# FrozenWolf-Cyber/Indic-CL-ASR

Measured on AMD Instinct MI355X. Metric: utterances/sec (15 s @16 kHz) Conformer-M RNNT-CTC+EWC train step, higher is better.
Workload: dtype bf16; 1 GPU; BASELINE configs[1]: Conformer-medium (d=256, 16L, H=640) hybrid RNNT-CTC + EWC, bs=32/GPU x 15 s, bf16 projections, freeze_encoder_till=12, 22x257 heads, fused_batch_size=4; global_batch=32, parallelism=dp1

## Files before the change

include/indicasr.h:

```cpp
#ifndef INDICASR_H
#define INDICASR_H

#include <stddef.h>
#include <stdint.h>

#ifdef __cplusplus
extern "C" {
#endif

typedef void* ia_stream_t;

enum ia_status {
    IA_OK = 0,
    IA_INVALID_VALUE = -1,
    IA_WORKSPACE_TOO_SMALL = -2,
    IA_LAUNCH_FAILED = -3,
    IA_UNSUPPORTED = -4,
};

const char* ia_version(void);

size_t ia_rnnt_workspace_bytes(int B, int T, int U1);
int ia_rnnt_loss(const float* logits, const int64_t* labels, const int64_t* act_lens, const int64_t* label_lens,
                 int B, int T, int U1, int V, int blank, float fastemit_lambda, float clamp,
// ... 6 lines not shown
                     const float* cost_grad, float* grads, void* workspace, size_t workspace_bytes, ia_stream_t stream,
                     void* grad_kernel_start_event, void* grad_kernel_stop_event);
int ia_rnnt_export_alphas_betas(const void* workspace, size_t workspace_bytes, const int64_t* act_lens,
                                const int64_t* label_lens, int B, int T, int U1, float* alphas, float* betas,
                                ia_stream_t stream);

int ia_joint_ld(int V);
int ia_joint_fwd(const void* f, const void* g, const void* W, const float* bias, const int64_t* labels,
                 const int64_t* act_lens, const int64_t* label_lens, int B, int T, int U1, int H, int V, int blank,
                 float dropout_p, unsigned seed, void* logits, int LD, void* workspace, size_t workspace_bytes,
                 ia_stream_t stream);
int ia_joint_fwd_box(const void* f, const void* g, const void* W, const float* bias, const int64_t* labels,
                     const int64_t* act_lens, const int64_t* label_lens, const int64_t* box_t, const int64_t* box_u, int B,
                     int T, int U1, int H, int V, int blank, float dropout_p, unsigned seed, void* logits, int LD,
                     void* workspace, size_t workspace_bytes, ia_stream_t stream);
int64_t ia_joint_extra_scratch_elems(void);
int ia_joint_extra_reduce(const void* logits, const void* teacher, const int64_t* box_t, const int64_t* box_u,
                          const float* w_sq, const float* w_kd, int B, int T, int U1, int V, int LD, float* sums4,
                          float* scratch, ia_stream_t stream);
int ia_joint_extra_grad(const void* logits, const void* teacher, const int64_t* box_t, const int64_t* box_u, const float* w_sq,
                        const float* w_kd, const float* upstream2, int B, int T, int U1, int V, int LD, void* E,
                        ia_stream_t stream);
int ia_lattice_add_f16(void* G, const void* E, int64_t n, ia_stream_t stream);
int ia_rnnt_lattice(const int64_t* act_lens, const int64_t* label_lens, int B, int T, int U1, float fastemit_lambda,
                    int need_backward, float* costs, void* workspace, size_t workspace_bytes, ia_stream_t stream);
int ia_joint_backward_g(void* logits_inout, const int64_t* labels, const int64_t* act_lens, const int64_t* label_lens,
                        int B, int T, int U1, int V, int LD, int blank, float fastemit_lambda, const float* cost_grad,
                        float kappa, void* gt_out, int S, int Kc, float* dbias_out, float* dbias_scratch, void* workspace,
                        size_t workspace_bytes, ia_stream_t stream, void* grad_kernel_start_event,
                        void* grad_kernel_stop_event);
int ia_joint_backward_g_skip(void* logits_inout, const int64_t* labels, const int64_t* act_lens, const int64_t* label_lens, int B,
                             int T, int U1, int V, int LD, int blank, float fastemit, const float* cost_grad, float kappa,
                             void* gt_out, int S, int Kc, float* dbias_out, float* dbias_scratch, void* workspace,
                             size_t workspace_bytes, int skip_dead_frames, ia_stream_t stream, void* ev_start, void* ev_stop);
int64_t ia_joint_backward_g_dbias_scratch_elems(int LD);
int ia_joint_hidden_t(const void* f, const void* g, void* hidden_t, int B, int T, int U1, int H, int LDH, int S, int Kc,
                      float dropout_p, unsigned seed, ia_stream_t stream);
int ia_joint_hidden(const void* f, const void* g, void* hidden, int B, int T, int U1, int H, int LDH, float dropout_p,
                    unsigned seed, ia_stream_t stream);
int ia_joint_dh_reduce(const void* dh, const void* f, const void* g, const int64_t* act_lens,
                       const int64_t* label_lens, float* df, float* dg, int B, int T, int U1, int H, float inv_kappa,
                       float dropout_p, unsigned seed, void* scratch, ia_stream_t stream);
size_t ia_joint_dh_reduce_scratch_bytes(int B, int T, int U1, int H);
int ia_joint_dh_fused_supported(int U1, int H, int LD);
int ia_joint_dh_k(void);
size_t ia_joint_dh_fused_scratch_bytes(int B, int T, int U1, int H);
int ia_joint_dh_fused(const void* G, const void* Wt, const void* f, const void* g, const int64_t* act_lens,
                      const int64_t* label_lens, float* df, float* dg, int B, int T, int U1, int H, int LD,
                      float inv_kappa, float dropout_p, unsigned seed, void* scratch, ia_stream_t stream);
int ia_joint_dh_fused_ex(const void* G, const void* Wt, const void* f, const void* g, const int64_t* act_lens,
                         const int64_t* label_lens, float* df, float* dg, void* df_bf16, void* dg_bf16, int zero_dead_df, int B,
                         int T, int U1, int H, int LD, float inv_kappa, float dropout_p, unsigned seed, void* scratch,
                         ia_stream_t stream);
int ia_joint_dw_fused_supported(int U1, int H, int LD);
int64_t ia_joint_dw_fused_scratch_elems(int B, int T, int U1, int H, int LD);
int ia_joint_dw_fused(const void* G, const void* f, const void* g, const int64_t* act_lens, int B, int T, int U1, int H, int LD,
                      float dropout_p, unsigned seed, float* dW, float* scratch, ia_stream_t stream);
int ia_joint_dw_fused_ex(const void* G, const void* f, const void* g, const int64_t* act_lens, const int64_t* label_lens, int B,
                         int T, int U1, int H, int LD, float dropout_p, unsigned seed, float* dW, float* scratch,
                         ia_stream_t stream);

int ia_gemm_bf16(const void* A, int lda, const void* W, int ldw, int M, int N, int K, const float* bias, int act,
                 float dropout_p, unsigned seed, float alpha, const float* R, int ldr, float* outF, int ldof,
                 void* outH, int ldoh, ia_stream_t stream);
int ia_gemm_bf16_ex(const void* A, int lda, const void* W, int ldw, int M, int N, int K, const float* bias, int act,
                    float dropout_p, unsigned seed, float alpha, const float* R, int ldr, float* outF, int ldof, void* outH,
                    int ldoh, void* out_pre, int ldpre, const void* aux, int ldaux, ia_stream_t stream);
int ia_gemm_bf16_ex2(const void* A, int lda, const void* W, int ldw, int M, int N, int K, const float* bias, int act,
                     float dropout_p, unsigned seed, float alpha, const float* R, int ldr, float* outF, int ldof, void* outH,
                     int ldoh, void* out_pre, int ldpre, const void* aux, int ldaux, int flags, ia_stream_t stream);
int ia_quantize_mxfp8(const void* x, int is_f32, int ld, int64_t M, int K, void* q, int ldq, void* scales, int lds, ia_stream_t stream);
int ia_gemm_mxfp8(const void* Aq, int lda, const void* a_scales, int ldsa, const void* Wq, int ldw, const void* w_scales, int ldsw,
                  int M, int N, int K, const float* bias, int act, float dropout_p, unsigned seed, float alpha, const float* R, int ldr,
                  float* outF, int ldof, void* outH, int ldoh, ia_stream_t stream);

int ia_greedy_decode_lds_bytes(int Hp, int Hj, int V);
int ia_greedy_rnnt_decode(const float* f_all, const int64_t* out_len, const float* EW, const float* Whh, const float* Wpred,
                          const float* bpred, const float* Whead, const float* bhead, int B, int T, int Hp, int Hj, int V,
                          int blank, int row_blank, int row_sos, int max_symbols, int* tokens, int cap, int* counts,
                          int* overflow, ia_stream_t stream);
int ia_greedy_rnnt_decode_bf16w(const float* f_all, const int64_t* out_len, const float* EW, const void* Whh_bf16,
                                const void* Wpred_bf16, const float* bpred, const void* Whead_bf16, const float* bhead, int B, int T,
                                int Hp, int Hj, int V, int blank, int row_blank, int row_sos, int max_symbols, int* tokens, int cap,
                                int* counts, int* overflow, ia_stream_t stream);
size_t ia_greedy_decode_scratch_bytes(int B, int Hp, int Hj);
int ia_greedy_decode_cluster(int B, int Hp, int Hj);
int ia_greedy_rnnt_decode_bf16w_ex(const float* f_all, const int64_t* out_len, const float* EW, const void* Whh_bf16,
                                   const void* Wpred_bf16, const float* bpred, const void* Whead_bf16, const float* bhead, int B,
                                   int T, int Hp, int Hj, int V, int blank, int row_blank, int row_sos, int max_symbols, int* tokens,
                                   int cap, int* counts, int* overflow, int cluster, void* scratch, size_t scratch_bytes,
                                   ia_stream_t stream);

int ia_edit_distance_batch(const int32_t* a, const int64_t* a_off, const int32_t* b, const int64_t* b_off, int n, int64_t* out);

int ia_quantize_fp8_rows(const void* x, int is_f32, int ld, int64_t M, int K, void* q, int ldq, float* scale, ia_stream_t stream);
int ia_gemm_fp8(const void* Aq, int lda, const float* a_scale, const void* Wq, int ldw, const float* w_scale, int M, int N, int K,
                const float* bias, int act, float dropout_p, unsigned seed, float alpha, const float* R, int ldr, float* outF,
                int ldof, void* outH, int ldoh, ia_stream_t stream);
int ia_subsample_conv1(const float* feats, int B, int Fm, int Tm, int C, const float* w1, const float* b1, void* out,
                       ia_stream_t stream);
int ia_subsample_conv2(const void* in_cl, int B, int T1, int F1, int C, const void* w2r, const float* b2, int N, void* out,
                       ia_stream_t stream);
int ia_gemm_bf16_ln_supported(int N, int K);
int ia_gemm_bf16_ln(const void* A, int lda, const void* W, int ldw, int M, int N, int K, const float* bias, float dropout_p,
                    unsigned seed, float alpha, const float* R, int ldr, float* outF, int ldof, const float* ln_g,
                    const float* ln_b, float ln_eps, void* outH, int ldoh, ia_stream_t stream);
// ... 450 lines not shown
```

indic_cl_asr_amd/_lib.py:

```python
import ctypes
import os
import subprocess

_HERE = os.path.dirname(os.path.abspath(__file__))
LIB_PATH = os.environ.get("IA_LIB_PATH") or os.path.join(_HERE, "libindicasr_hip.so")

IA_OK = 0
_STATUS = {-1: "IA_INVALID_VALUE", -2: "IA_WORKSPACE_TOO_SMALL", -3: "IA_LAUNCH_FAILED", -4: "IA_UNSUPPORTED"}

_c = ctypes
_vp, _i, _f, _sz = _c.c_void_p, _c.c_int, _c.c_float, _c.c_size_t
_i64 = _c.c_int64

class BlockParams(_c.Structure):
    _fields_ = ([(n, _c.c_void_p) for n in (
        "w_ff1a", "w_ff1b", "w_qkv", "w_pos", "w_out", "w_pw1", "w_pw2", "w_ff2a", "w_ff2b",
        "b_ff1a", "b_ff1b", "b_qkv", "b_out", "b_pw1", "b_pw2", "b_ff2a", "b_ff2b",
        "ln_ff1_g", "ln_ff1_b", "ln_att_g", "ln_att_b", "ln_conv_g", "ln_conv_b", "ln_ff2_g", "ln_ff2_b", "ln_out_g", "ln_out_b",
        "pos_u", "pos_v", "dw_w", "dw_b", "bn_g", "bn_b", "bn_rm", "bn_rv", "bn_nbt")]
        + [(n, _c.c_float) for n in ("ln_eps", "bn_eps", "bn_momentum", "p_drop", "p_ff", "p_att", "fc_factor")]
        + [(n, _c.c_int) for n in ("d", "d_ff", "n_heads", "ksz")]
        + [("pl_cached", _c.c_void_p), ("w_pw1_glu", _c.c_void_p), ("b_pw1_glu", _c.c_void_p), ("att_window", _c.c_int),
           ("att_style", _c.c_int), ("att_left", _c.c_int), ("att_right", _c.c_int)])

# ... 52 lines not shown
    "ia_rnnt_backward": (_i, [_vp, _vp, _vp, _vp, _i, _i, _i, _i, _i, _f, _f, _vp, _vp, _vp, _sz, _vp, _vp, _vp]),
    "ia_rnnt_export_alphas_betas": (_i, [_vp, _sz, _vp, _vp, _i, _i, _i, _vp, _vp, _vp]),
    "ia_joint_ld": (_i, [_i]),
    "ia_joint_fwd": (_i, [_vp, _vp, _vp, _vp, _vp, _vp, _vp, _i, _i, _i, _i, _i, _i, _f, _c.c_uint, _vp, _i, _vp, _sz, _vp]),
    "ia_joint_fwd_box": (_i, [_vp, _vp, _vp, _vp, _vp, _vp, _vp, _vp, _vp, _i, _i, _i, _i, _i, _i, _f, _c.c_uint, _vp, _i, _vp, _sz, _vp]),
    "ia_joint_extra_scratch_elems": (_i64, []),
    "ia_joint_extra_reduce": (_i, [_vp, _vp, _vp, _vp, _vp, _vp, _i, _i, _i, _i, _i, _vp, _vp, _vp]),
    "ia_joint_extra_grad": (_i, [_vp, _vp, _vp, _vp, _vp, _vp, _vp, _i, _i, _i, _i, _i, _vp, _vp]),
    "ia_lattice_add_f16": (_i, [_vp, _vp, _i64, _vp]),
    "ia_relpos_attention_flash_lse": (_i, [_vp, _vp, _vp, _vp, _vp, _i, _i, _i, _i, _f, _c.c_uint, _vp, _vp, _vp]),
    "ia_relpos_attention_flash_bwd_dims": (_i, [_i, _c.POINTER(_c.c_int), _c.POINTER(_c.c_int)]),
    "ia_relpos_attention_flash_bwd_ws_elems": (_i64, [_i, _i, _i, _i]),
    "ia_relpos_attention_flash_bwd": (_i, [_vp, _vp, _vp, _vp, _vp, _vp, _vp, _vp, _i, _i, _i, _i, _f, _c.c_uint, _vp, _vp, _i, _vp,
                                           _vp, _vp, _vp, _vp, _vp]),
    "ia_relpos_attention_local_lse": (_i, [_vp, _vp, _vp, _vp, _vp, _i, _i, _i, _i, _i, _f, _c.c_uint, _vp, _vp, _vp]),
    "ia_relpos_attention_local_bwd_dims": (_i, [_i, _i, _c.POINTER(_c.c_int), _c.POINTER(_c.c_int)]),
    "ia_relpos_attention_local_bwd_ws_elems": (_i64, [_i, _i, _i, _i, _i]),
    "ia_relpos_attention_local_bwd": (_i, [_vp, _vp, _vp, _vp, _vp, _vp, _vp, _vp, _i, _i, _i, _i, _i, _f, _c.c_uint, _vp, _vp, _i, _vp,
                                           _vp, _vp, _vp, _vp, _vp]),
    "ia_relpos_attention_context_lse": (_i, [_vp, _vp, _vp, _vp, _vp, _i, _i, _i, _i, _i, _i, _i, _f, _c.c_uint, _vp, _vp, _vp]),
    "ia_relpos_attention_context_bwd_dims": (_i, [_i, _i, _i, _i, _c.POINTER(_c.c_int), _c.POINTER(_c.c_int)]),
    "ia_relpos_attention_context_bwd_ws_elems": (_i64, [_i, _i, _i, _i, _i, _i, _i]),
    "ia_relpos_attention_context_bwd": (_i, [_vp, _vp, _vp, _vp, _vp, _vp, _vp, _vp, _i, _i, _i, _i, _i, _i, _i, _f, _c.c_uint, _vp, _vp,
                                             _i, _vp, _vp, _vp, _vp, _vp, _vp]),
    "ia_quantize_fp8_rows": (_i, [_vp, _i, _i, _i64, _i, _vp, _i, _vp, _vp]),
    "ia_gemm_fp8": (_i, [_vp, _i, _vp, _vp, _i, _vp, _i, _i, _i, _vp, _i, _f, _c.c_uint, _f, _vp, _i, _vp, _i, _vp, _i, _vp]),
    "ia_gemm_tn_grouped_scratch_elems": (_i64, [_vp, _i]),
    "ia_gemm_tn_bf16_grouped": (_i, [_vp, _i, _vp, _vp]),
    "ia_greedy_decode_lds_bytes": (_i, [_i, _i, _i]),
    "ia_greedy_rnnt_decode": (_i, [_vp, _vp, _vp, _vp, _vp, _vp, _vp, _vp, _i, _i, _i, _i, _i, _i, _i, _i, _i, _vp, _i, _vp, _vp, _vp]),
    "ia_greedy_rnnt_decode_bf16w": (_i, [_vp, _vp, _vp, _vp, _vp, _vp, _vp, _vp, _i, _i, _i, _i, _i, _i, _i, _i, _i, _vp, _i, _vp, _vp, _vp]),
    "ia_edit_distance_batch": (_i, [_vp, _vp, _vp, _vp, _i, _vp]),
    "ia_greedy_decode_scratch_bytes": (_sz, [_i, _i, _i]),
    "ia_greedy_decode_cluster": (_i, [_i, _i, _i]),
    "ia_greedy_rnnt_decode_bf16w_ex": (_i, [_vp, _vp, _vp, _vp, _vp, _vp, _vp, _vp, _i, _i, _i, _i, _i, _i, _i, _i, _i, _vp, _i, _vp, _vp, _i, _vp, _sz, _vp]),
    "ia_quantize_mxfp8": (_i, [_vp, _i, _i, _i64, _i, _vp, _i, _vp, _i, _vp]),
    "ia_gemm_mxfp8": (_i, [_vp, _i, _vp, _i, _vp, _i, _vp, _i, _i, _i, _i, _vp, _i, _f, _c.c_uint, _f, _vp, _i, _vp, _i, _vp, _i, _vp]),
    "ia_cast_pad_bf16": (_i, [_vp, _i, _i64, _i, _vp, _i, _vp]),
    "ia_rnnt_lattice": (_i, [_vp, _vp, _i, _i, _i, _f, _i, _vp, _vp, _sz, _vp]),
    "ia_joint_backward_g": (_i, [_vp, _vp, _vp, _vp, _i, _i, _i, _i, _i, _i, _f, _vp, _f, _vp, _i, _i, _vp, _vp, _vp, _sz, _vp, _vp,
                                 _vp]),
    "ia_joint_backward_g_skip": (_i, [_vp, _vp, _vp, _vp, _i, _i, _i, _i, _i, _i, _f, _vp, _f, _vp, _i, _i, _vp, _vp, _vp, _sz, _i, _vp,
                                      _vp, _vp]),
    "ia_joint_backward_g_dbias_scratch_elems": (_i64, [_i]),
    "ia_joint_hidden_t": (_i, [_vp, _vp, _vp, _i, _i, _i, _i, _i, _i, _i, _f, _c.c_uint, _vp]),
    "ia_joint_hidden": (_i, [_vp, _vp, _vp, _i, _i, _i, _i, _i, _f, _c.c_uint, _vp]),
    "ia_joint_dh_reduce": (_i, [_vp, _vp, _vp, _vp, _vp, _vp, _vp, _i, _i, _i, _i, _f, _f, _c.c_uint, _vp, _vp]),
    "ia_joint_dh_reduce_scratch_bytes": (_sz, [_i, _i, _i, _i]),
    "ia_joint_dh_fused_supported": (_i, [_i, _i, _i]),
    "ia_joint_dh_k": (_i, []),
    "ia_joint_dh_fused": (_i, [_vp, _vp, _vp, _vp, _vp, _vp, _vp, _vp, _i, _i, _i, _i, _i, _f, _f, _c.c_uint, _vp, _vp]),
    "ia_joint_dh_fused_ex": (_i, [_vp, _vp, _vp, _vp, _vp, _vp, _vp, _vp, _vp, _vp, _i, _i, _i, _i, _i, _i, _f, _f, _c.c_uint, _vp, _vp]),
    "ia_joint_dh_fused_scratch_bytes": (_sz, [_i, _i, _i, _i]),
    "ia_joint_dw_fused_supported": (_i, [_i, _i, _i]),
    "ia_joint_dw_fused_scratch_elems": (_i64, [_i, _i, _i, _i, _i]),
    "ia_joint_dw_fused": (_i, [_vp, _vp, _vp, _vp, _i, _i, _i, _i, _i, _f, _c.c_uint, _vp, _vp, _vp]),
    "ia_gemm_bf16_ln_supported": (_i, [_i, _i]),
    "ia_gemm_bf16_ln": (_i, [_vp, _i, _vp, _i, _i, _i, _i, _vp, _f, _c.c_uint, _f, _vp, _i, _vp, _i, _vp, _vp, _f, _vp, _i, _vp]),
    "ia_joint_dw_fused_ex": (_i, [_vp, _vp, _vp, _vp, _vp, _i, _i, _i, _i, _i, _f, _c.c_uint, _vp, _vp, _vp]),
    "ia_gemm_bf16": (_i, [_vp, _i, _vp, _i, _i, _i, _i, _vp, _i, _f, _c.c_uint, _f, _vp, _i, _vp, _i, _vp, _i, _vp]),
    "ia_gemm_bf16_ex": (_i, [_vp, _i, _vp, _i, _i, _i, _i, _vp, _i, _f, _c.c_uint, _f, _vp, _i, _vp, _i, _vp, _i, _vp, _i, _vp, _i, _vp]),
    "ia_subsample_conv1": (_i, [_vp, _i, _i, _i, _i, _vp, _vp, _vp, _vp]),
    "ia_subsample_conv2": (_i, [_vp, _i, _i, _i, _i, _vp, _vp, _i, _vp, _vp]),
    "ia_layernorm": (_i, [_vp, _i, _i, _i, _vp, _vp, _f, _vp, _i, _vp, _vp, _vp, _i, _vp]),
    "ia_glu_dwconv": (_i, [_vp, _vp, _i, _i, _i, _i, _vp, _vp, _vp, _vp, _vp, _vp, _vp]),
    "ia_dwconv_scratch_elems": (_i64, [_i, _i, _i, _i]),
    "ia_colsum_bf16": (_i, [_vp, _i, _i, _i, _vp, _vp]),
    "ia_dwconv_time": (_i, [_vp, _i, _i, _i, _i, _vp, _vp, _i, _vp, _vp]),
    "ia_dwconv_time_wgrad": (_i, [_vp, _vp, _i, _i, _i, _i, _vp, _vp, _vp, _vp]),
    "ia_dwconv_glu_bwd": (_i, [_vp, _vp, _vp, _i, _i, _i, _i, _vp, _vp, _vp]),
    "ia_dwconv_glu_wgrad": (_i, [_vp, _vp, _vp, _i, _i, _i, _i, _vp, _vp, _vp, _vp]),
    "ia_bn_silu": (_i, [_vp, _i64, _i, _vp, _vp, _vp, _vp, _vp, _vp, _vp, _f, _f, _i, _vp, _vp]),
    "ia_gemm_bnsilu_supported": (_i, [_i]),
    "ia_gemm_bnsilu_bf16": (_i, [_vp, _i, _i64, _vp, _vp, _vp, _vp, _vp, _vp, _vp, _f, _f, _i, _vp, _i, _i, _i, _i, _vp, _f, _c.c_uint, _f,
                                 _vp, _i, _vp, _i, _vp, _i, _vp, _vp]),
    "ia_gemm_bnsilu_bf16_keep": (_i, [_vp, _i, _i64, _vp, _vp, _vp, _vp, _vp, _vp, _vp, _f, _f, _i, _vp, _i, _i, _i, _i, _vp, _f, _c.c_uint,
                                      _f, _vp, _i, _vp, _i, _vp, _i, _vp, _vp, _i, _vp]),
    "ia_glu_dwconv_fixed": (_i, [_vp, _vp, _i, _i, _i, _i, _vp, _vp, _vp, _vp, _vp]),
    "ia_dwconv_gated_fixed": (_i, [_vp, _vp, _i, _i, _i, _i, _vp, _vp, _vp, _vp, _vp]),
    "ia_attn_vt_elems": (_sz, [_i, _i, _i]),
    "ia_relpos_attention": (_i, [_vp, _vp, _vp, _vp, _vp, _i, _i, _i, _i, _f, _c.c_uint, _vp, _vp, _vp]),
    "ia_relpos_attention_flash_supported": (_i, [_i, _i]),
    "ia_relpos_attention_flash": (_i, [_vp, _vp, _vp, _vp, _vp, _i, _i, _i, _i, _f, _c.c_uint, _vp, _vp]),
    "ia_relpos_attention_local_supported": (_i, [_i, _i, _i]),
    "ia_relpos_attention_context_supported": (_i, [_i, _i, _i, _i, _i]),
    "ia_relpos_attention_context": (_i, [_vp, _vp, _vp, _vp, _vp, _i, _i, _i, _i, _i, _i, _i, _f, _c.c_uint, _vp, _vp]),
    "ia_relpos_attention_local": (_i, [_vp, _vp, _vp, _vp, _vp, _i, _i, _i, _i, _i, _f, _c.c_uint, _vp, _vp]),
    "ia_lstm_scratch_bytes": (_sz, [_i, _i]),
    "ia_lstm_lds_bytes": (_i, [_i, _i]),
    "ia_lstm_forward": (_i, [_vp, _vp, _vp, _vp, _vp, _i, _i, _i, _vp, _sz, _vp]),
    "ia_lstm_backward": (_i, [_vp, _vp, _vp, _vp, _vp, _i, _i, _i, _vp, _sz, _vp]),
    "ia_feat_frames": (_i, [_vp, _i, _i, _i, _i, _i, _i, _f, _f, _c.c_uint, _vp, _i, _vp]),
    "ia_gemm_f32": (_i, [_vp, _i, _vp, _i, _i, _i, _i, _vp, _i, _vp]),
    "ia_feat_power": (_i, [_vp, _i64, _i, _i, _i, _vp, _i, _vp]),
    "ia_feat_logmel_t": (_i, [_vp, _i, _i, _i, _i, _f, _vp, _vp]),
    "ia_feat_preemph": (_i, [_vp, _i, _i, _f, _f, _c.c_uint, _vp, _vp]),
    "ia_feat_logmel_fft_supported": (_i, [_i, _i, _i, _i]),
    "ia_feat_logmel_fft": (_i, [_vp, _i, _i, _i, _vp, _i, _i, _i, _vp, _vp, _vp, _vp, _i, _i, _f, _vp, _vp]),
    "ia_feat_normalize": (_i, [_vp, _vp, _i, _i, _i, _f, _vp, _vp, _i, _vp, _vp, _i, _f, _vp, _vp]),
    "ia_ctc_workspace_bytes": (_sz, [_i, _i, _i]),
    "ia_ctc_forward": (_i, [_vp, _vp, _vp, _vp, _i, _i, _i, _i, _i, _i, _vp, _vp, _sz, _vp]),
    "ia_ctc_backward": (_i, [_vp, _vp, _vp, _vp, _i, _i, _i, _i, _i, _vp, _vp, _vp, _sz, _vp]),
    "ia_ctc_align_max_targets": (_i, []),
    "ia_ctc_align_workspace_bytes": (_sz, [_i, _i, _i]),
    "ia_ctc_align": (_i, [_vp, _i, _vp, _vp, _vp, _vp, _i, _i, _i, _i, _i, _vp, _vp, _vp, _vp, _sz, _vp]),
    "ia_ctc_beam_max_width": (_i, []),
# ... 139 lines not shown
```

indic_cl_asr_amd/csrc/joint_dh.hip:

```cpp
#include <hip/hip_bf16.h>
#include <stdio.h>
#include <stdlib.h>

#include "joint_common.h"

namespace {

constexpr int DH_KP = 288;
constexpr int DH_KS = DH_KP / 32;
constexpr int DH_AROW = DH_KP * 2 + 16;
constexpr int DH_ROWS = 64;
constexpr int DH_NB_MAX = 384;
constexpr int DH_TT = 16;

struct DhArgs {
    const _Float16* G; const _Float16* Wt; const _Float16* f; const _Float16* g;
    const int64_t* act_lens; const int64_t* label_lens;
    float* df; float* part;
    __bf16* dfb;
    int B, T, U1, H, LD, nh;
    float inv_kappa;
    unsigned seed, thr;
    int diag;
};

__device__ __forceinline__ void dh_mfma(f4& acc, const h8& a_frag, const h8& b_frag) {
    asm("v_mfma_f32_16x16x32_f16 %0, %1, %2, %0" : "+v"(acc) : "v"(a_frag), "a"(b_frag));
}

#define DH_TIE_ACC5                                                                                                 \
    "+v"(acc[0][0]), "+v"(acc[0][1]), "+v"(acc[0][2]), "+v"(acc[0][3]), "+v"(acc[0][4]), "+v"(acc[1][0]), "+v"(acc[1][1]),  \
        "+v"(acc[1][2]), "+v"(acc[1][3]), "+v"(acc[1][4]), "+v"(acc[2][0]), "+v"(acc[2][1]), "+v"(acc[2][2]), "+v"(acc[2][3]), \
        "+v"(acc[2][4]), "+v"(acc[3][0]), "+v"(acc[3][1]), "+v"(acc[3][2]), "+v"(acc[3][3]), "+v"(acc[3][4])
#define DH_TIE_ACC2                                                                                                 \
    "+v"(acc[0][0]), "+v"(acc[0][1]), "+v"(acc[1][0]), "+v"(acc[1][1]), "+v"(acc[2][0]), "+v"(acc[2][1]), "+v"(acc[3][0]), "+v"(acc[3][1])

template <int NT>
__device__ __forceinline__ void dh_multiply(f4 (&acc)[4][NT], const unsigned char* sAl, const h8 (&Bf)[NT][DH_KS], bool skip) {
    static_assert(NT == 5 || NT == 2, "the accumulator tie lists are written out for 5 and 2 column tiles");
#pragma unroll
    for (int mt = 0; mt < 4; ++mt)
#pragma unroll
        for (int nt = 0; nt < NT; ++nt) acc[mt][nt] = (f4){0.f, 0.f, 0.f, 0.f};
    if constexpr (NT == 5) { asm volatile("s_nop 4" : DH_TIE_ACC5); } else { asm volatile("s_nop 4" : DH_TIE_ACC2); }
    if (!skip) {
        h8 Af[2][4];
#pragma unroll
        for (int mt = 0; mt < 4; ++mt) Af[0][mt] = *reinterpret_cast<const h8*>(sAl + mt * 16 * DH_AROW);
#pragma unroll
        for (int ks = 0; ks < DH_KS; ++ks) {
            if (ks + 1 < DH_KS) {
#pragma unroll
                for (int mt = 0; mt < 4; ++mt)
                    Af[(ks + 1) & 1][mt] = *reinterpret_cast<const h8*>(sAl + mt * 16 * DH_AROW + (ks + 1) * 64);
            }
#pragma unroll
            for (int nt = 0; nt < NT; ++nt)
#pragma unroll
                for (int mt = 0; mt < 4; ++mt)
                    dh_mfma(acc[mt][nt], Af[ks & 1][mt], Bf[nt][ks]);
        }
    }
    if constexpr (NT == 5) { asm volatile("s_nop 15\n\ts_nop 15" : DH_TIE_ACC5); } else { asm volatile("s_nop 15\n\ts_nop 15" : DH_TIE_ACC2); }
}

template <int WAVES>
__device__ __forceinline__ void dh_load_g_rows(unsigned char* dst, const _Float16* G, int b, int T, int U1, int LD, int t_first, int u_first,
                                               int wave, int lane, int diag) {
    constexpr int SLOTS = DH_AROW / 16, NBLK = (DH_ROWS * SLOTS + 63) / 64;
    const int vpr = LD / 8;
    for (int blk = wave; blk < NBLK; blk += WAVES) {
        const int P = blk * 64 + lane;
        const int row = P / SLOTS, col = P - row * SLOTS;
        int t = t_first + (row >> 4); t = t < T ? t : T - 1;
        int u = u_first + (row & 15); u = u < U1 ? u : U1 - 1;
        const _Float16* src = G + (((size_t)b * T + t) * U1 + u) * LD + col * 8;
        if (row < DH_ROWS && col < vpr && !(diag & 4))
            ia_lds_dma16(reinterpret_cast<const unsigned char*>(src), dst + blk * 1024);
    }
}

template <bool DROPOUT, int DH_NT, int DH_WAVES>
__global__ __launch_bounds__(DH_WAVES * 64, (DH_WAVES + 3) / 4) void joint_dh_fused_kernel(DhArgs a) {
    constexpr int DH_NW = 16 * DH_NT;
    constexpr int DH_NB = DH_NW * DH_WAVES;
    constexpr int DH_THREADS = DH_WAVES * 64;
    static_assert(DH_NB <= DH_NB_MAX, "d f accumulator rows");
    extern __shared__ __attribute__((aligned(16))) unsigned char smem[];
    unsigned char* sA = smem;
    float* sdf = reinterpret_cast<float*>(smem + 2 * DH_ROWS * DH_AROW);
    unsigned char* smask = reinterpret_cast<unsigned char*>(sdf + DH_TT * DH_NB);
    const int tid = threadIdx.x, lane = tid & 63, wave = tid >> 6;
    const int c = lane & 15, q = lane >> 4;
    const int T = a.T, U1 = a.U1, H = a.H, LD = a.LD;
    const int ntt = (T + DH_TT - 1) / DH_TT;
    int bid = blockIdx.x;
    int half;
    {
        const int ntiles = (int)gridDim.x / a.nh, full = (ntiles / 8) * 8;
        const int grp = bid / (8 * a.nh), r = bid - grp * (8 * a.nh);
        if (grp * 8 < full) { half = r >> 3; bid = grp * 8 + (r & 7); }
        else { const int r2 = bid - full * a.nh; half = r2 % a.nh; bid = full + r2 / a.nh; }
    }
    const int tt = bid % ntt;
    const int b = bid / ntt;
    const int t0 = tt * DH_TT;
    int Tb = (int)a.act_lens[b]; Tb = Tb < T ? Tb : T;
    int Ub = (int)a.label_lens[b] + 1; Ub = Ub < U1 ? Ub : U1;
    if (t0 >= Tb) return;
    const int nut = (Ub + 15) / 16;
    int npt = (Tb - t0 + 3) / 4; npt = npt < 4 ? npt : 4;
    const int n0 = half * DH_NB + wave * DH_NW;
    const bool wave_on = n0 < H;

    h8 Bf[DH_NT][DH_KS];
    {
        const int nb = wave_on ? n0 : 0;
#pragma unroll
        for (int nt = 0; nt < DH_NT; ++nt)
#pragma unroll
            for (int ks = 0; ks < DH_KS; ++ks)
                Bf[nt][ks] = *reinterpret_cast<const h8*>(a.Wt + (size_t)(nb + nt * 16 + c) * DH_KP + ks * 32 + q * 8);
    }
    for (int i = tid; i < 2 * DH_ROWS * DH_AROW / 16; i += DH_THREADS) reinterpret_cast<uint4*>(sA)[i] = make_uint4(0, 0, 0, 0);
    for (int i = tid; i < DH_TT * DH_NB; i += DH_THREADS) sdf[i] = 0.f;
    __syncthreads();

    unsigned char* smw = smask + wave * 1024;
    float dgacc[4][DH_NT];
    _Float16 gh[4][DH_NT];
    auto begin_label_tile = [&](int u0) {
#pragma unroll
        for (int r = 0; r < 4; ++r) {
            int u = u0 + q * 4 + r; u = u < U1 ? u : U1 - 1;
            const _Float16* gp = a.g + ((size_t)b * U1 + u) * H + n0 + c;
#pragma unroll
            for (int nt = 0; nt < DH_NT; ++nt) { gh[r][nt] = gp[nt * 16]; dgacc[r][nt] = 0.f; }
        }
    };
    auto load_f_rows = [&](int tp, _Float16 (&fh)[4][DH_NT]) {
#pragma unroll
        for (int mt = 0; mt < 4; ++mt) {
            int t = tp + mt; t = t < T ? t : T - 1;
            const _Float16* fp = a.f + ((size_t)b * T + t) * H + n0 + c;
#pragma unroll
            for (int nt = 0; nt < DH_NT; ++nt) fh[mt][nt] = fp[nt * 16];
        }
    };
    auto fill_keep_table = [&](int tp, int u0) {
#pragma unroll
        for (int i = 0; i < 2 * DH_NT; ++i) {
            const int e = lane + 64 * i, row = e / (2 * DH_NT), j = e - row * (2 * DH_NT);
            const int nt = j >> 1, cp = j & 1;
            const int tr = tp + (row >> 4), ur = u0 + (row & 15);
            const unsigned cell = (unsigned)((((size_t)b * T + tr) * U1) + ur);
            unsigned bits = 0xFFu;
            if (DROPOUT) bits = dropout_keep8(a.seed, cell, (unsigned)((n0 >> 3) + j), a.thr);
            smw[row * 16 + cp * 8 + nt] = (unsigned char)((tr < T && ur < U1) ? bits : 0u);
        }
    };
    auto store_dg_partial = [&](int u0) {
#pragma unroll
        for (int r = 0; r < 4; ++r) {
            const int u = u0 + q * 4 + r;
            if (u < U1) {
                float* pp = a.part + ((((size_t)b * ntt + tt) * U1) + u) * H + n0 + c;
#pragma unroll
                for (int nt = 0; nt < DH_NT; ++nt) pp[nt * 16] = dgacc[r][nt];
            }
        }
    };

    const int npass = nut * npt;
    dh_load_g_rows<DH_WAVES>(sA, a.G, b, T, U1, LD, t0, 0, wave, lane, a.diag);
    ia_lds_dma_wait();
    __syncthreads();
#pragma unroll
    for (int r = 0; r < 4; ++r)
#pragma unroll
// ... 113 lines not shown
            const int64_t b = i / frow4, r = i - b * frow4;
            const int t = (int)(r / (H / 4));
            int Tb = (int)act_lens[b]; Tb = Tb < T ? Tb : T;
            const int tlive = (Tb + DH_TT - 1) / DH_TT * DH_TT;
            if (t >= tlive) {
                if (df) reinterpret_cast<float4*>(df)[i] = make_float4(0.f, 0.f, 0.f, 0.f);
                if (dfb) reinterpret_cast<uint2*>(dfb)[i] = make_uint2(0u, 0u);
            }
        }
    }
}
template <bool DROPOUT, int NT, int WAVES>
int dh_launch(DhArgs a, hipStream_t st) {
    constexpr int nb = 16 * NT * WAVES;
    constexpr size_t lds = 2 * (size_t)DH_ROWS * DH_AROW + (size_t)DH_TT * nb * sizeof(float) + (size_t)WAVES * 1024;
    a.nh = (a.H + nb - 1) / nb;
    const int ntt = (a.T + DH_TT - 1) / DH_TT;
    IA_SET_MAX_LDS_ONCE((joint_dh_fused_kernel<DROPOUT, NT, WAVES>), (int)lds);
    hipLaunchKernelGGL((joint_dh_fused_kernel<DROPOUT, NT, WAVES>), dim3((unsigned)(a.B * ntt * a.nh)), dim3(WAVES * 64), lds, st, a);
    const hipError_t e = hipGetLastError();
    if (e != hipSuccess) {
        if (getenv("IA_DEBUG")) {
            hipFuncAttributes fa;
            const hipError_t e2 = hipFuncGetAttributes(&fa, (const void*)joint_dh_fused_kernel<DROPOUT, NT, WAVES>);
            fprintf(stderr, "ia_joint_dh_fused: launch failed: %s (waves %d, lds %zu; attr rc %d maxThreadsPerBlock %d numRegs %d "
                            "maxDynShared %d sharedSizeBytes %zu localSizeBytes %zu)\n", hipGetErrorString(e), WAVES, lds, (int)e2,
                    fa.maxThreadsPerBlock, fa.numRegs, fa.maxDynamicSharedSizeBytes, fa.sharedSizeBytes, fa.localSizeBytes);
        }
        return IA_LAUNCH_FAILED;
    }
    return IA_OK;
}
}

extern "C" int ia_joint_dh_fused_supported(int U1, int H, int LD) {
    return (U1 >= 1 && H >= 80 && H % 80 == 0 && LD % 8 == 0 && LD >= 8 && LD <= DH_KP) ? 1 : 0;
}

extern "C" int ia_joint_dh_k(void) { return DH_KP; }

extern "C" size_t ia_joint_dh_fused_scratch_bytes(int B, int T, int U1, int H) {
    if (B <= 0 || T <= 0 || U1 <= 0 || H <= 0) return 0;
    return (size_t)B * ((T + DH_TT - 1) / DH_TT) * U1 * H * sizeof(float);
}

extern "C" int ia_joint_dh_fused(const void* G, const void* Wt, const void* f, const void* g, const int64_t* act_lens,
                                 const int64_t* label_lens, float* df, float* dg, int B, int T, int U1, int H, int LD,
                                 float inv_kappa, float dropout_p, unsigned seed, void* scratch, ia_stream_t stream) {
    if (!df || !dg) return IA_INVALID_VALUE;
    return ia_joint_dh_fused_ex(G, Wt, f, g, act_lens, label_lens, df, dg, nullptr, nullptr, 0, B, T, U1, H, LD, inv_kappa, dropout_p, seed,
                                scratch, stream);
}

extern "C" int ia_joint_dh_fused_ex(const void* G, const void* Wt, const void* f, const void* g, const int64_t* act_lens,
                                    const int64_t* label_lens, float* df, float* dg, void* df_bf16, void* dg_bf16, int zero_dead_df,
                                    int B, int T, int U1, int H, int LD, float inv_kappa, float dropout_p, unsigned seed,
                                    void* scratch, ia_stream_t stream) {
    if (!G || !Wt || !f || !g || !act_lens || !label_lens || (!df && !df_bf16) || (!dg && !dg_bf16) || !scratch || B <= 0 || T <= 0)
        return IA_INVALID_VALUE;
    if (!ia_joint_dh_fused_supported(U1, H, LD)) return IA_UNSUPPORTED;
    if (!ia_is_aligned(G, 16) || !ia_is_aligned(Wt, 16) || (dg && !ia_is_aligned(dg, 16)) || (df && !ia_is_aligned(df, 16)) ||
        (df_bf16 && !ia_is_aligned(df_bf16, 16)) || (dg_bf16 && !ia_is_aligned(dg_bf16, 16)) || !ia_is_aligned(scratch, 16) ||
        dropout_p < 0.f || dropout_p >= 1.f || H % 4 != 0)
        return IA_INVALID_VALUE;
    DhArgs a;
    a.G = (const _Float16*)G; a.Wt = (const _Float16*)Wt; a.f = (const _Float16*)f; a.g = (const _Float16*)g;
    a.act_lens = act_lens; a.label_lens = label_lens; a.df = df; a.dfb = (__bf16*)df_bf16; a.part = (float*)scratch;
    { const char* e = getenv("IA_DH_DIAG"); a.diag = e ? atoi(e) : 0; }
    a.B = B; a.T = T; a.U1 = U1; a.H = H; a.LD = LD;
    a.nh = 0;
    a.inv_kappa = inv_kappa; a.seed = seed;
    a.thr = ia_dropout_rule(dropout_p).thr;
    const char* wv_env = getenv("IA_DH_WAVES");
    const bool ten = H % 32 == 0 && !(wv_env && atoi(wv_env) == 4);
    hipStream_t st = (hipStream_t)stream;
    const int rc = ten ? (a.thr > 0 ? dh_launch<true, 2, 10>(a, st) : dh_launch<false, 2, 10>(a, st))
                       : (a.thr > 0 ? dh_launch<true, 5, 4>(a, st) : dh_launch<false, 5, 4>(a, st));
    if (rc != IA_OK) return rc;
    const int64_t n4 = (int64_t)B * U1 * H / 4;
    const int fgrid = (int)((n4 + 255) / 256 < 8192 ? (n4 + 255) / 256 : 8192);
    hipLaunchKernelGGL(joint_dh_dg_finish_kernel, dim3(fgrid < 1 ? 1 : fgrid), dim3(256), 0, st, (const float*)scratch, dg,
                       (__bf16*)dg_bf16, df, (__bf16*)df_bf16, zero_dead_df ? 1 : 0, act_lens, label_lens, B, T, U1, H, inv_kappa);
    IA_RETURN_IF_LAUNCH_FAILED();
    return IA_OK;
}
```

Measured before the change: 3787 utterances/s.

## Schedule joint dh workgroups longest-first via on-device cost histogram ordering

```diff
diff --git a/include/indicasr.h b/include/indicasr.h
--- a/include/indicasr.h
+++ b/include/indicasr.h
@@ -82,6 +82,13 @@
                          const int64_t* label_lens, float* df, float* dg, void* df_bf16, void* dg_bf16, int zero_dead_df, int B,
                          int T, int U1, int H, int LD, float inv_kappa, float dropout_p, unsigned seed, void* scratch,
                          ia_stream_t stream);
+int ia_joint_dh_order_supported(int B, int U1);
+int ia_joint_dh_order(const int64_t* act_lens_host, const int64_t* label_lens_host, int B, int T, int U1, int* b_out, int* tt_out);
+int ia_joint_dh_items(int B, int T, int H);
+int ia_joint_dh_fused_items(const void* G, const void* Wt, const void* f, const void* g, const int64_t* act_lens,
+                            const int64_t* label_lens, float* df, float* dg, void* df_bf16, void* dg_bf16, int zero_dead_df, int B,
+                            int T, int U1, int H, int LD, float inv_kappa, float dropout_p, unsigned seed, void* scratch, int* items,
+                            ia_stream_t stream);
 int ia_joint_dw_fused_supported(int U1, int H, int LD);
 int64_t ia_joint_dw_fused_scratch_elems(int B, int T, int U1, int H, int LD);
 int ia_joint_dw_fused(const void* G, const void* f, const void* g, const int64_t* act_lens, int B, int T, int U1, int H, int LD,
diff --git a/indic_cl_asr_amd/_lib.py b/indic_cl_asr_amd/_lib.py
--- a/indic_cl_asr_amd/_lib.py
+++ b/indic_cl_asr_amd/_lib.py
@@ -128,6 +128,10 @@
     "ia_joint_dh_fused": (_i, [_vp, _vp, _vp, _vp, _vp, _vp, _vp, _vp, _i, _i, _i, _i, _i, _f, _f, _c.c_uint, _vp, _vp]),
     "ia_joint_dh_fused_ex": (_i, [_vp, _vp, _vp, _vp, _vp, _vp, _vp, _vp, _vp, _vp, _i, _i, _i, _i, _i, _i, _f, _f, _c.c_uint, _vp, _vp]),
     "ia_joint_dh_fused_scratch_bytes": (_sz, [_i, _i, _i, _i]),
+    "ia_joint_dh_order_supported": (_i, [_i, _i]),
+    "ia_joint_dh_order": (_i, [_vp, _vp, _i, _i, _i, _vp, _vp]),
+    "ia_joint_dh_items": (_i, [_i, _i, _i]),
+    "ia_joint_dh_fused_items": (_i, [_vp, _vp, _vp, _vp, _vp, _vp, _vp, _vp, _vp, _vp, _i, _i, _i, _i, _i, _i, _f, _f, _c.c_uint, _vp, _vp, _vp]),
     "ia_joint_dw_fused_supported": (_i, [_i, _i, _i]),
     "ia_joint_dw_fused_scratch_elems": (_i64, [_i, _i, _i, _i, _i]),
     "ia_joint_dw_fused": (_i, [_vp, _vp, _vp, _vp, _i, _i, _i, _i, _i, _f, _c.c_uint, _vp, _vp, _vp]),
diff --git a/indic_cl_asr_amd/csrc/joint_dh.hip b/indic_cl_asr_amd/csrc/joint_dh.hip
--- a/indic_cl_asr_amd/csrc/joint_dh.hip
+++ b/indic_cl_asr_amd/csrc/joint_dh.hip
@@ -3,6 +3,7 @@
 #include <stdlib.h>
 
 #include "joint_common.h"
+#include "joint_dh_order.h"
 
 namespace {
 
@@ -22,7 +23,36 @@
     float inv_kappa;
     unsigned seed, thr;
     int diag;
+    int order;
+    int* items;
 };
+
+__device__ __forceinline__ void dh_order_resolve(int* tab, int j, const int64_t* act_lens, const int64_t* label_lens, int B, int T, int U1, int lane) {
+    const int nkeys = dh_order_nkeys(U1);
+    int* hist = tab;
+    int* utt = tab + DH_ORD_HIST_INTS;
+    int* res = tab + DH_ORD_TABLE_INTS;
+    for (int k = lane; k < dh_order_pad(nkeys); k += 64) hist[k] = 0;
+    __builtin_amdgcn_fence(__ATOMIC_ACQ_REL, "wavefront");
+    __builtin_amdgcn_wave_barrier();
+    for (int b0 = 0; b0 < dh_order_pad(B); b0 += 64) {
+        const int b = b0 + lane, bc = b < B ? b : B - 1;
+        const int64_t al = act_lens[bc], ll = label_lens[bc];
+        const int on = -(int)(b < B);
+        const int Tb = dh_order_frames(al, T) & on, nut = dh_order_label_tiles(ll, U1) & on;
+        if (b < dh_order_pad(B)) {
+            const DhOrderUtt u = dh_order_utt(Tb, nut);
+            if (u.nfull) atomicAdd(&hist[u.kfull], u.nfull);
+            if (u.kpart != DH_ORD_NO_KEY) atomicAdd(&hist[u.kpart], 1);
+            utt[2 * b] = Tb;
+            utt[2 * b + 1] = nut;
+        }
+    }
+    __builtin_amdgcn_fence(__ATOMIC_ACQ_REL, "wavefront");
+    __builtin_amdgcn_wave_barrier();
+    const DhOrderItem it = dh_order_find(j, hist, utt, B, nkeys);
+    if (lane == 0) { res[0] = it.b; res[1] = it.tt; res[2] = it.Tb; res[3] = it.nut; }
+}
 
 __device__ __forceinline__ void dh_mfma(f4& acc, const h8& a_frag, const h8& b_frag) {
     asm("v_mfma_f32_16x16x32_f16 %0, %1, %2, %0" : "+v"(acc) : "v"(a_frag), "a"(b_frag));
@@ -86,6 +116,7 @@
     constexpr int DH_NB = DH_NW * DH_WAVES;
     constexpr int DH_THREADS = DH_WAVES * 64;
     static_assert(DH_NB <= DH_NB_MAX, "d f accumulator rows");
+    static_assert(DH_TT == DH_ORD_TT && (DH_ORD_TABLE_INTS + 8) * sizeof(int) <= DH_WAVES * 1024, "the order's table lives in the keep tables' LDS");
     extern __shared__ __attribute__((aligned(16))) unsigned char smem[];
     unsigned char* sA = smem;
     float* sdf = reinterpret_cast<float*>(smem + 2 * DH_ROWS * DH_AROW);
@@ -102,14 +133,18 @@
         if (grp * 8 < full) { half = r >> 3; bid = grp * 8 + (r & 7); }
         else { const int r2 = bid - full * a.nh; half = r2 % a.nh; bid = full + r2 / a.nh; }
     }
-    const int tt = bid % ntt;
-    const int b = bid / ntt;
-    const int t0 = tt * DH_TT;
-    int Tb = (int)a.act_lens[b]; Tb = Tb < T ? Tb : T;
-    int Ub = (int)a.label_lens[b] + 1; Ub = Ub < U1 ? Ub : U1;
-    if (t0 >= Tb) return;
-    const int nut = (Ub + 15) / 16;
-    int npt = (Tb - t0 + 3) / 4; npt = npt < 4 ? npt : 4;
+    int b_ = bid / ntt, tt_ = bid % ntt, Tb_ = 0, nut_ = 0;
+    if (!a.order) {
+        Tb_ = (int)a.act_lens[b_]; Tb_ = Tb_ < T ? Tb_ : T;
+        int Ub = (int)a.label_lens[b_] + 1; Ub = Ub < U1 ? Ub : U1;
+        nut_ = (Ub + 15) / 16;
+        if (tt_ * DH_TT >= Tb_) {
+            if (a.items && tid == 0) a.items[3 * blockIdx.x] = -1;
+            return;
+        }
+    } else if (wave == 0) {
+        dh_order_resolve(reinterpret_cast<int*>(smask), bid, a.act_lens, a.label_lens, a.B, T, U1, lane);
+    }
     const int n0 = half * DH_NB + wave * DH_NW;
     const bool wave_on = n0 < H;
 
@@ -125,6 +160,19 @@
     for (int i = tid; i < 2 * DH_ROWS * DH_AROW / 16; i += DH_THREADS) reinterpret_cast<uint4*>(sA)[i] = make_uint4(0, 0, 0, 0);
     for (int i = tid; i < DH_TT * DH_NB; i += DH_THREADS) sdf[i] = 0.f;
     __syncthreads();
+    if (a.order) {
+        const int4 res = *reinterpret_cast<const int4*>(reinterpret_cast<const int*>(smask) + DH_ORD_TABLE_INTS);
+        b_ = __builtin_amdgcn_readfirstlane(res.x); tt_ = __builtin_amdgcn_readfirstlane(res.y);
+        Tb_ = __builtin_amdgcn_readfirstlane(res.z); nut_ = __builtin_amdgcn_readfirstlane(res.w);
+        if (b_ < 0) {
+            if (a.items && tid == 0) a.items[3 * blockIdx.x] = -1;
+            return;
+        }
+    }
+    const int b = b_, tt = tt_, Tb = Tb_, nut = nut_;
+    const int t0 = tt * DH_TT;
+    if (a.items && tid == 0) { a.items[3 * blockIdx.x] = b; a.items[3 * blockIdx.x + 1] = tt; a.items[3 * blockIdx.x + 2] = half; }
+    int npt = (Tb - t0 + 3) / 4; npt = npt < 4 ? npt : 4;
 
     unsigned char* smw = smask + wave * 1024;
     float dgacc[4][DH_NT];
@@ -344,10 +392,10 @@
                                 scratch, stream);
 }
 
-extern "C" int ia_joint_dh_fused_ex(const void* G, const void* Wt, const void* f, const void* g, const int64_t* act_lens,
-                                    const int64_t* label_lens, float* df, float* dg, void* df_bf16, void* dg_bf16, int zero_dead_df,
-                                    int B, int T, int U1, int H, int LD, float inv_kappa, float dropout_p, unsigned seed,
-                                    void* scratch, ia_stream_t stream) {
+namespace {
+int dh_fused(const void* G, const void* Wt, const void* f, const void* g, const int64_t* act_lens, const int64_t* label_lens, float* df,
+             float* dg, void* df_bf16, void* dg_bf16, int zero_dead_df, int B, int T, int U1, int H, int LD, float inv_kappa,
+             float dropout_p, unsigned seed, void* scratch, int* items, ia_stream_t stream) {
     if (!G || !Wt || !f || !g || !act_lens || !label_lens || (!df && !df_bf16) || (!dg && !dg_bf16) || !scratch || B <= 0 || T <= 0)
         return IA_INVALID_VALUE;
     if (!ia_joint_dh_fused_supported(U1, H, LD)) return IA_UNSUPPORTED;
@@ -361,6 +409,8 @@
     { const char* e = getenv("IA_DH_DIAG"); a.diag = e ? atoi(e) : 0; }
     a.B = B; a.T = T; a.U1 = U1; a.H = H; a.LD = LD;
     a.nh = 0;
+    { const char* e = getenv("IA_DH_ORDER"); a.order = !(e && atoi(e) == 0) && dh_order_supported(B, U1) ? 1 : 0; }
+    a.items = items;
     a.inv_kappa = inv_kappa; a.seed = seed;
     a.thr = ia_dropout_rule(dropout_p).thr;
     const char* wv_env = getenv("IA_DH_WAVES");
@@ -376,3 +426,51 @@
     IA_RETURN_IF_LAUNCH_FAILED();
     return IA_OK;
 }
+}
+
+extern "C" int ia_joint_dh_fused_ex(const void* G, const void* Wt, const void* f, const void* g, const int64_t* act_lens,
+                                    const int64_t* label_lens, float* df, float* dg, void* df_bf16, void* dg_bf16, int zero_dead_df,
+                                    int B, int T, int U1, int H, int LD, float inv_kappa, float dropout_p, unsigned seed,
+                                    void* scratch, ia_stream_t stream) {
+    return dh_fused(G, Wt, f, g, act_lens, label_lens, df, dg, df_bf16, dg_bf16, zero_dead_df, B, T, U1, H, LD, inv_kappa, dropout_p, seed,
+                    scratch, nullptr, stream);
+}
+
+extern "C" int ia_joint_dh_fused_items(const void* G, const void* Wt, const void* f, const void* g, const int64_t* act_lens,
+                                       const int64_t* label_lens, float* df, float* dg, void* df_bf16, void* dg_bf16, int zero_dead_df,
+                                       int B, int T, int U1, int H, int LD, float inv_kappa, float dropout_p, unsigned seed,
+                                       void* scratch, int* items, ia_stream_t stream) {
+    if (!items) return IA_INVALID_VALUE;
+    return dh_fused(G, Wt, f, g, act_lens, label_lens, df, dg, df_bf16, dg_bf16, zero_dead_df, B, T, U1, H, LD, inv_kappa, dropout_p, seed,
+                    scratch, items, stream);
+}
+
+extern "C" int ia_joint_dh_items(int B, int T, int H) {
+    if (B <= 0 || T <= 0 || H <= 0) return 0;
+    static_assert(16 * 5 * 4 == 320 && 16 * 2 * 10 == 320, "both decompositions cover 320 hidden units per workgroup");
+    return B * ((T + DH_TT - 1) / DH_TT) * ((H + 319) / 320);
+}
+
+extern "C" int ia_joint_dh_order_supported(int B, int U1) { return dh_order_supported(B, U1) ? 1 : 0; }
+
+extern "C" int ia_joint_dh_order(const int64_t* act_lens_host, const int64_t* label_lens_host, int B, int T, int U1, int* b_out, int* tt_out) {
+    if (!act_lens_host || !label_lens_host || !b_out || !tt_out || B <= 0 || T <= 0 || U1 <= 0) return IA_INVALID_VALUE;
+    const int ntt = (T + DH_TT - 1) / DH_TT;
+    int n = 0;
+    if (!dh_order_supported(B, U1)) {
+        for (int b = 0; b < B; ++b)
+            for (int tt = 0; tt < ntt && tt * DH_TT < dh_order_frames(act_lens_host[b], T); ++tt) { b_out[n] = b; tt_out[n] = tt; ++n; }
+        return n;
+    }
+    int* tab = (int*)malloc(sizeof(int) * DH_ORD_TABLE_INTS);
+    if (!tab) return IA_INVALID_VALUE;
+    const int live = dh_order_build_host(act_lens_host, label_lens_host, B, T, U1, tab, tab + DH_ORD_HIST_INTS);
+    for (; n < live; ++n) {
+        const DhOrderItem it = dh_order_find(n, tab, tab + DH_ORD_HIST_INTS, B, dh_order_nkeys(U1));
+        if (it.b < 0) break;
+        b_out[n] = it.b;
+        tt_out[n] = it.tt;
+    }
+    free(tab);
+    return n == live ? live : IA_INVALID_VALUE;
+}
diff --git a/indic_cl_asr_amd/csrc/joint_dh_order.h b/indic_cl_asr_amd/csrc/joint_dh_order.h
--- /dev/null
+++ b/indic_cl_asr_amd/csrc/joint_dh_order.h
@@ -0,0 +1,89 @@
+#pragma once
+#include <stdint.h>
+
+namespace {
+
+constexpr int DH_ORD_TT = 16;
+constexpr int DH_ORD_MAX_B = 256;
+constexpr int DH_ORD_MAX_KEYS = 257;
+constexpr int DH_ORD_NO_KEY = -1;
+constexpr int DH_ORD_STEP = 8;
+constexpr int DH_ORD_HIST_INTS = (DH_ORD_MAX_KEYS + DH_ORD_STEP - 1) / DH_ORD_STEP * DH_ORD_STEP;
+constexpr int DH_ORD_TABLE_INTS = DH_ORD_HIST_INTS + 2 * DH_ORD_MAX_B;
+
+__host__ __device__ inline int dh_order_pad(int n) { return (n + DH_ORD_STEP - 1) / DH_ORD_STEP * DH_ORD_STEP; }
+__host__ __device__ inline int dh_order_nkeys(int U1) { return 4 * ((U1 + 15) / 16) + 1; }
+__host__ __device__ inline bool dh_order_supported(int B, int U1) {
+    return B >= 1 && B <= DH_ORD_MAX_B && U1 >= 1 && dh_order_nkeys(U1) <= DH_ORD_MAX_KEYS;
+}
+
+__host__ __device__ inline int dh_order_frames(int64_t act_len, int T) { return act_len < (int64_t)T ? (int)(act_len < 0 ? 0 : act_len) : T; }
+__host__ __device__ inline int dh_order_label_tiles(int64_t label_len, int U1) {
+    const int64_t ub = label_len + 1 < (int64_t)U1 ? label_len + 1 : (int64_t)U1;
+    return ub < 1 ? 0 : (int)((ub + 15) / 16);
+}
+
+static_assert(DH_ORD_TT == 16, "dh_order_utt shifts by 4");
+struct DhOrderUtt { int nfull, kfull, kpart; };
+__host__ __device__ inline DhOrderUtt dh_order_utt(int Tb, int nut) {
+    DhOrderUtt u;
+    const int rem = Tb & (DH_ORD_TT - 1);
+    u.nfull = Tb >> 4;
+    u.kfull = 4 * nut;
+    u.kpart = rem ? nut * ((rem + 3) >> 2) : DH_ORD_NO_KEY;
+    return u;
+}
+
+struct DhOrderItem { int b, tt, Tb, nut; };
+__host__ __device__ inline DhOrderItem dh_order_find(int j, const int* hist, const int* utt, int B, int nkeys) {
+    int before = 0, key = -1, r = 0;
+    for (int k0 = dh_order_pad(nkeys) - DH_ORD_STEP; k0 >= 0; k0 -= DH_ORD_STEP) {
+        int h[DH_ORD_STEP];
+#pragma unroll
+        for (int i = 0; i < DH_ORD_STEP; ++i) h[i] = hist[k0 + i];
+#pragma unroll
+        for (int i = DH_ORD_STEP - 1; i >= 0; --i) {
+            const bool hit = j >= before && j < before + h[i];
+            key = hit ? k0 + i : key;
+            r = hit ? j - before : r;
+            before += h[i];
+        }
+    }
+    DhOrderItem it = {-1, 0, 0, 0};
+    if (key < 0) return it;
+    int p = 0;
+    for (int b0 = 0; b0 < B; b0 += DH_ORD_STEP) {
+        int Tb[DH_ORD_STEP], nut[DH_ORD_STEP];
+#pragma unroll
+        for (int i = 0; i < DH_ORD_STEP; ++i) { Tb[i] = utt[2 * (b0 + i)]; nut[i] = utt[2 * (b0 + i) + 1]; }
+#pragma unroll
+        for (int i = 0; i < DH_ORD_STEP; ++i) {
+            const DhOrderUtt u = dh_order_utt(Tb[i], nut[i]);
+            const int cf = u.kfull == key ? u.nfull : 0;
+            const int c = cf + (u.kpart == key ? 1 : 0);
+            const bool hit = r >= p && r < p + c;
+            it.b = hit ? b0 + i : it.b;
+            it.tt = hit ? (r - p < cf ? r - p : u.nfull) : it.tt;
+            it.Tb = hit ? Tb[i] : it.Tb;
+            it.nut = hit ? nut[i] : it.nut;
+            p += c;
+        }
+    }
+    return it;
+}
+
+inline int dh_order_build_host(const int64_t* act_lens, const int64_t* label_lens, int B, int T, int U1, int* hist, int* utt) {
+    for (int k = 0; k < dh_order_pad(dh_order_nkeys(U1)); ++k) hist[k] = 0;
+    int live = 0;
+    for (int b = 0; b < dh_order_pad(B); ++b) {
+        const int Tb = b < B ? dh_order_frames(act_lens[b], T) : 0, nut = b < B ? dh_order_label_tiles(label_lens[b], U1) : 0;
+        const DhOrderUtt u = dh_order_utt(Tb, nut);
+        hist[u.kfull] += u.nfull;
+        if (u.kpart != DH_ORD_NO_KEY) hist[u.kpart] += 1;
+        utt[2 * b] = Tb;
+        utt[2 * b + 1] = nut;
+        live += u.nfull + (u.kpart != DH_ORD_NO_KEY ? 1 : 0);
+    }
+    return live;
+}
+}
```

Result: no change. 3784 utterances/s (-0.1%).
